# microsoft/DirectXTex

Hardware: AMD Instinct MI355X
Metric: Mtexels/s BC7 encode (4096^2 RGBA8, TEX_COMPRESS_DEFAULT) (higher is better)
Workload: dtype fp32 seed fit + i32 exact error sums (u8 texels in, 128-bit blocks out); 1 GPU; cfg2: 4096x4096 RGBA8 -> BC7_UNORM, TEX_COMPRESS_DEFAULT, one image per GPU, source and payload resident in HBM (dxtex_compress_device)

## Files before the change

### directxtex_amd/csrc/bc6h_encode.hip

```cpp
#include "dxtex_kernels.h"
#include "bc67_tables.h"
#include "bc7_core.h"
#include "bc6h_core.h"
#include "search_common.h"
#include <algorithm>
#include <cstdlib>
#include <cstdio>
#include <vector>

namespace dxtex
{
namespace
{
using namespace bc6h;

struct Ep16 { uint32_t a01, a2b0, b12; };
__device__ __forceinline__ Ep16 pack_ep16(const int (&A)[3], const int (&B)[3])
{
    Ep16 e;
    e.a01 = (uint32_t(A[0]) & 0xFFFFu) | (uint32_t(A[1]) << 16);
    e.a2b0 = (uint32_t(A[2]) & 0xFFFFu) | (uint32_t(B[0]) << 16);
    e.b12 = (uint32_t(B[1]) & 0xFFFFu) | (uint32_t(B[2]) << 16);
    return e;
}
// ... 976 lines not shown
        const uint32_t myTask = a.order[idx].x;
        const Rec6 rec = a.recs[myTask];
        const uint32_t nb = myTask % a.nblocks;
        const int prec = a.prec1[myTask / a.nblocks];
        const float* gp = a.fpix + uint64_t(nb) * 48 + (lane & 15);
        const float tr = gp[0], tg = gp[16], tb = gp[32];
        EndPts e;
        unpack_ep16(rec.ep, sg, e.A, e.B);
        Perturb6 st = perturb6_begin(e, rec.err);
        while (st.ch < 3)
        {
            float err; int v;
            perturb6_wave_macro(tr, tg, tb, lane, st, prec, sg, err, v);
            st = perturb6_transition(st, err, v);
        }
        if (lane == 0)
        {
            a.recs[myTask].ep = pack_ep16(st.ep.A, st.ep.B);
            { const float mk = ep16_mark(sg, st.ep.A, st.ep.B); if (mk < 0.0f) a.recs[myTask].err = mk; }
        }
    }
}

__global__ void __launch_bounds__(256) bc6h_store_kernel(Bc6hArgs a)
{
    const uint32_t nb = blockIdx.x * 256u + threadIdx.x;
    if (nb >= a.nblocks) return;
    const Best6 b = a.best[nb];
    const BcSeg& im = seg_of(a.seg, nb);
    const uint32_t gb = im.nb0 + (nb - im.l0);
    const uint32_t by = gb / im.nbw, bx = gb - by * im.nbw;
    uint64_t* out = reinterpret_cast<uint64_t*>(im.dst + uint64_t(by) * im.dstRowPitch) + 2 * uint64_t(bx);
    out[0] = b.lo; out[1] = b.hi;
}

const uint64_t kMaxBlocksPerPass6 = dev_env("DXTEX_MAX_BLOCKS_PER_PASS") ? std::max<uint64_t>(1, strtoull(dev_env("DXTEX_MAX_BLOCKS_PER_PASS"), nullptr, 10)) : (1u << 22);
struct Scratch6
{
    size_t fpix, lists, seeds, recs, orgs, order, tinfo, counters, best, bounds, recs1, orgs1, order1, tinfo1, counters1, opts, total;
    explicit Scratch6(uint64_t nb)
    {
        auto up = [](size_t v) { return (v + 255) & ~size_t(255); };
        size_t o = 0;
        fpix = o; o = up(o + nb * 48 * sizeof(float));
        lists = o; o = up(o + nb * 8);
        seeds = o; o = up(o + nb * SEED_INTS * sizeof(int));
        recs = o; o = up(o + nb * 16 * sizeof(Rec6));
        orgs = o; o = up(o + nb * 16 * sizeof(OrgSave));
        order = o; o = up(o + nb * 16 * sizeof(uint2));
        tinfo = o; o = up(o + nb * 16 * sizeof(uint32_t));
        counters = o; o = up(o + 128 * sizeof(uint32_t));
        best = o; o = up(o + nb * sizeof(Best6));
        bounds = o; o = up(o + nb * 17 * sizeof(float));
        recs1 = o; o = up(o + nb * 4 * sizeof(Rec6));
        orgs1 = o; o = up(o + nb * 4 * sizeof(OrgSave));
        order1 = o; o = up(o + nb * 4 * sizeof(uint2));
        tinfo1 = o; o = up(o + nb * 4 * sizeof(uint32_t));
        counters1 = o; o = up(o + 128 * sizeof(uint32_t));
        opts = o; o = up(o + nb * 16 * sizeof(OptSave));
        total = o;
    }
};
}

size_t bc6h_scratch_bytes(uint64_t nblocks, size_t nimages)
{
    return Scratch6(nblocks < kMaxBlocksPerPass6 ? nblocks : kMaxBlocksPerPass6).total + seg_table_bytes(nblocks, kMaxBlocksPerPass6, nimages);
}

hipError_t launch_bc6h_encode(const SrcView& src, uint8_t* dst, uint64_t dstRowPitch, bool isSigned, void* scratch,
                              hipStream_t stream, KernelMarks* marks, const SideStreams* side)
{
    BcImage one; one.src = src; one.dst = dst; one.dstRowPitch = dstRowPitch;
    return launch_bc6h_encode_many(&one, 1, isSigned, scratch, stream, marks, side);
}

hipError_t launch_bc6h_encode_many(const BcImage* images, size_t count, bool isSigned, void* scratch, hipStream_t stream, KernelMarks* marks,
                                   const SideStreams* side)
{
#define DXTEX_MARK(NAME) do { if (marks) marks->mark(NAME); } while (0)
    std::vector<BcSeg> segs;
    std::vector<BcPass> passes;
    uint64_t perPass = 0;
    if (!build_passes(images, count, kMaxBlocksPerPass6, segs, passes, &perPass)) return hipSuccess;
    const Scratch6 L(perPass);
    uint8_t* base = static_cast<uint8_t*>(scratch);
    BcSeg* dSegs = reinterpret_cast<BcSeg*>(base + L.total);
    const hipError_t ce = upload_segments(dSegs, segs, passes, stream);
    if (ce != hipSuccess) return ce;
    for (const BcPass& pass : passes)
    {
        Bc6hArgs a;
        set_pass(a.seg, dSegs, segs, pass);
        a.nblocks = pass.nblocks;
        a.isSigned = isSigned ? 1 : 0;
        static const bool noPrune = dev_env("DXTEX_BC6H_NO_PRUNE") != nullptr;
        a.prune = noPrune ? 0 : 1;
        a.fpix = reinterpret_cast<float*>(base + L.fpix);
        a.lists = base + L.lists;
        a.seeds = reinterpret_cast<int*>(base + L.seeds);
        a.recs = reinterpret_cast<Rec6*>(base + L.recs);
        a.orgs = reinterpret_cast<OrgSave*>(base + L.orgs);
        a.order = reinterpret_cast<uint2*>(base + L.order);
        a.tinfo = reinterpret_cast<uint32_t*>(base + L.tinfo);
        a.counters = reinterpret_cast<uint32_t*>(base + L.counters);
        a.best = reinterpret_cast<Best6*>(base + L.best);
        a.bounds = reinterpret_cast<float*>(base + L.bounds);
        a.opts = reinterpret_cast<OptSave*>(base + L.opts);
        a.saveOpt = 0;
        a.boundsReady = 0;
        a.filterStats = 0;
        a.mode = ModeRt();

        DXTEX_MARK("bc6h_rough");
        hipLaunchKernelGGL(bc6h_rough_kernel, dim3((a.nblocks + 3) / 4), dim3(256), 0, stream, a);
        DXTEX_MARK("bc6h_block_seed");
        hipLaunchKernelGGL(bc6h_block_seed_kernel, dim3((a.nblocks + 255) / 256), dim3(256), 0, stream, a);
        if (dev_env("DXTEX_BC6H_DUMP"))
        {
            (void)hipStreamSynchronize(stream);
            const uint32_t n = std::min<uint32_t>(a.nblocks, 4);
            std::vector<uint8_t> l(n * 8); std::vector<int> sd(n * SEED_INTS);
            (void)hipMemcpy(l.data(), a.lists, l.size(), hipMemcpyDeviceToHost);
            (void)hipMemcpy(sd.data(), a.seeds, sd.size() * 4, hipMemcpyDeviceToHost);
            for (uint32_t b = 0; b < n; ++b)
            {
                fprintf(stderr, "block %u shapes:", b);
                for (int i = 0; i < 8; ++i) fprintf(stderr, " %d", l[b * 8 + i]);
                fprintf(stderr, "\n  seeds rank0:");
                for (int i = 0; i < 12; ++i) fprintf(stderr, " %d", sd[b * SEED_INTS + i]);
                fprintf(stderr, "\n");
            }
        }
        static const int onlyMode = dev_env("DXTEX_BC6H_ONLY_MODE") ? atoi(dev_env("DXTEX_BC6H_ONLY_MODE")) : -1;
        static const bool noSearch = dev_env("DXTEX_BC6H_NO_SEARCH") != nullptr;
        static const Bc6hMode kModes[14] = {
            { 0x00, 1, 1, 3, { 10, 10, 10 }, { 5, 5, 5 } }, { 0x01, 1, 1, 3, { 7, 7, 7 }, { 6, 6, 6 } }, { 0x02, 1, 1, 3, { 11, 11, 11 }, { 5, 4, 4 } },
            { 0x06, 1, 1, 3, { 11, 11, 11 }, { 4, 5, 4 } }, { 0x0a, 1, 1, 3, { 11, 11, 11 }, { 4, 4, 5 } }, { 0x0e, 1, 1, 3, { 9, 9, 9 }, { 5, 5, 5 } },
            { 0x12, 1, 1, 3, { 8, 8, 8 }, { 6, 5, 5 } }, { 0x16, 1, 1, 3, { 8, 8, 8 }, { 5, 6, 5 } }, { 0x1a, 1, 1, 3, { 8, 8, 8 }, { 5, 5, 6 } },
            { 0x1e, 1, 0, 3, { 6, 6, 6 }, { 6, 6, 6 } }, { 0x03, 0, 0, 4, { 10, 10, 10 }, { 10, 10, 10 } }, { 0x07, 0, 1, 4, { 11, 11, 11 }, { 9, 9, 9 } },
            { 0x0b, 0, 1, 4, { 12, 12, 12 }, { 8, 8, 8 } }, { 0x0f, 0, 1, 4, { 16, 16, 16 }, { 4, 4, 4 } } };
        auto set_mode_on = [&](Bc6hArgs& a, int mi)
        {
            const Bc6hMode& k = kModes[mi];
            a.mode.index = mi; a.mode.code = k.code; a.mode.regions2 = k.regions2; a.mode.transformed = k.transformed; a.mode.prec = k.prec[0];
            for (int c = 0; c < 3; ++c) a.mode.delta[c] = k.delta[c];
        };
        auto set_mode = [&](int mi) { set_mode_on(a, mi); };
        auto sort_tasks = [&](const Bc6hArgs& a, uint32_t ntasks, hipStream_t stream)
        {
            const uint32_t binGroups = std::min<uint32_t>(kBinGroups, (ntasks + 255) / 256);
            (void)hipMemsetAsync(a.counters, 0, 128 * sizeof(uint32_t), stream);
            hipLaunchKernelGGL(bc7_bin_count_kernel, dim3(binGroups), dim3(256), 0, stream, a.tinfo, ntasks, a.counters);
            hipLaunchKernelGGL(bc7_bin_scan_kernel, dim3(1), dim3(1), 0, stream, a.counters);
            hipLaunchKernelGGL(bc7_bin_scatter_kernel, dim3(binGroups), dim3(256), 0, stream, a.tinfo, ntasks, a.counters, a.order);
        };
        a.taskBase = 0;
        for (int m = 0; m < 4; ++m) a.prec1[m] = kModes[10 + m].prec[0];
        static const std::vector<int> order6 = []
        {
            std::vector<int> o;
            const char* e = dev_env("DXTEX_BC6H_ORDER");
            const char* p = e ? e : DXTEX_BC6H_DEFAULT_ORDER;
            while (*p) { if (*p >= '0' && *p <= '9') o.push_back(int(strtol(p, const_cast<char**>(&p), 10))); else ++p; }
            return o;
        }();
        int prevPrec = -1;
        a.samePrec = 0;
        std::vector<int> run2;
        for (int mi : order6) if (mi >= 0 && mi <= 9 && (onlyMode < 0 || mi == onlyMode)) run2.push_back(mi);
        static const int forkBack = dev_env("DXTEX_BC6H_FORK_BACK") ? atoi(dev_env("DXTEX_BC6H_FORK_BACK")) : 2;
        const SideStreams* fork = (marks || forkBack <= 0 || run2.size() < size_t(forkBack) + 1 || onlyMode >= 0) ? nullptr : side;
        Bc6hArgs a1 = a;
        a1.recs = reinterpret_cast<Rec6*>(base + L.recs1);
        a1.orgs = reinterpret_cast<OrgSave*>(base + L.orgs1);
        a1.order = reinterpret_cast<uint2*>(base + L.order1);
        a1.tinfo = reinterpret_cast<uint32_t*>(base + L.tinfo1);
        a1.counters = reinterpret_cast<uint32_t*>(base + L.counters1);
        a1.samePrec = 0;
        auto one_region_search = [&](hipStream_t stream, KernelMarks* marks)
        {
            const uint32_t gridPP = (a1.nblocks + 255) / 256;
            DXTEX_MARK("bc6h_pre_1region");
            a1.boundsReady = 0;
            for (int m = 0; m < 4; ++m)
            {
                if (onlyMode >= 0 && 10 + m != onlyMode) continue;
                set_mode_on(a1, 10 + m); a1.taskBase = uint32_t(m) * a1.nblocks;
                hipLaunchKernelGGL(bc6h_pre_kernel<0>, dim3(gridPP), dim3(256), 0, stream, a1);
                a1.boundsReady = 1;
            }
            const uint32_t ntasks = a1.nblocks * 4u;
            if (onlyMode >= 0)
                for (int m = 0; m < 4; ++m) if (10 + m != onlyMode) (void)hipMemsetAsync(a1.tinfo + uint64_t(m) * a1.nblocks, 0, uint64_t(a1.nblocks) * 4, stream);
            DXTEX_MARK("bc6h_bin_1region");
            sort_tasks(a1, ntasks, stream);
            DXTEX_MARK("bc6h_perturb_1region");
            static const uint32_t waveMax = dev_env("DXTEX_BC6H_WAVE_MAX") ? uint32_t(strtoul(dev_env("DXTEX_BC6H_WAVE_MAX"), nullptr, 0)) : kWaveTaskMax6;
            if (!noSearch)
            {
                hipLaunchKernelGGL(bc6h_perturb_kernel<16>, dim3(std::min<uint32_t>(kSearchWaves, (ntasks + 63) / 64)), dim3(64), 0, stream, a1, waveMax);
                hipLaunchKernelGGL(bc6h_perturb_wave_kernel, dim3(std::min<uint32_t>(kSearchWaves, ntasks)), dim3(64), 0, stream, a1, waveMax);
            }
        };
        bool forked = false;
        for (size_t at = 0; at < run2.size(); ++at)
        {
            const int mi = run2[at];
            if (fork && at + size_t(forkBack) == run2.size())
            {
                (void)hipEventRecord(fork->forked, stream);
                (void)hipStreamWaitEvent(fork->side[0], fork->forked, 0);
                one_region_search(fork->side[0], nullptr);
                (void)hipEventRecord(fork->joined[0], fork->side[0]);
                forked = true;
            }
            set_mode(mi);
            static const bool noReuse = dev_env("DXTEX_BC6H_NO_REUSE") != nullptr;
            a.samePrec = (!noReuse && prevPrec == kModes[mi].prec[0]) ? 1 : 0;
            prevPrec = kModes[mi].prec[0];
            a.saveOpt = (!noReuse && at + 1 < run2.size() && kModes[run2[at + 1]].prec[0] == kModes[mi].prec[0]) ? 1 : 0;
            const uint32_t ntasks = a.nblocks * 16u;
            const uint32_t gridPP = (a.nblocks + 15) / 16;
            static const char* const kPre[10] = { "bc6h_pre_m0", "bc6h_pre_m1", "bc6h_pre_m2", "bc6h_pre_m3", "bc6h_pre_m4", "bc6h_pre_m5", "bc6h_pre_m6", "bc6h_pre_m7", "bc6h_pre_m8", "bc6h_pre_m9" };
            static const char* const kPerturb[10] = { "bc6h_perturb_m0", "bc6h_perturb_m1", "bc6h_perturb_m2", "bc6h_perturb_m3", "bc6h_perturb_m4", "bc6h_perturb_m5", "bc6h_perturb_m6", "bc6h_perturb_m7", "bc6h_perturb_m8", "bc6h_perturb_m9" };
            static const char* const kPost[10] = { "bc6h_post_m0", "bc6h_post_m1", "bc6h_post_m2", "bc6h_post_m3", "bc6h_post_m4", "bc6h_post_m5", "bc6h_post_m6", "bc6h_post_m7", "bc6h_post_m8", "bc6h_post_m9" };
            DXTEX_MARK(kPre[mi]);
            hipLaunchKernelGGL(bc6h_pre_kernel<1>, dim3(gridPP), dim3(256), 0, stream, a);
            a.boundsReady = 1;
            DXTEX_MARK("bc6h_bin_2region");
            sort_tasks(a, ntasks, stream);
#if defined(DXTEX_DEV)
            static const bool stats6 = dev_env("DXTEX_BC6H_STATS") != nullptr;
            a.filterStats = stats6 ? 1 : 0;
            if (stats6)
            {
                uint32_t c[40] = {};
                (void)hipStreamSynchronize(stream);
                (void)hipMemcpy(c, a.counters, sizeof(c), hipMemcpyDeviceToHost);
                std::fprintf(stderr, "bc6h stats mode %d (prec %d): %u task slots, %u live (16-texel: %u)\n", mi, a.mode.prec, ntasks, c[34], c[16]);
            }
#endif
            DXTEX_MARK(kPerturb[mi]);
            static const bool plainPerturb = dev_env("DXTEX_BC6H_PERTURB_PLAIN") != nullptr;
            if (!noSearch)
            {
                const dim3 grid(std::min<uint32_t>(kSearchWaves, (ntasks + 63) / 64));
                if (plainPerturb) hipLaunchKernelGGL(bc6h_perturb_kernel<8>, grid, dim3(64), 0, stream, a, 0u);
                else if (isSigned) hipLaunchKernelGGL(bc6h_perturb_filter_kernel<true>, grid, dim3(64), 0, stream, a);
                else hipLaunchKernelGGL(bc6h_perturb_filter_kernel<false>, grid, dim3(64), 0, stream, a);
            }
#if defined(DXTEX_DEV)
            if (stats6 && !plainPerturb)
            {
                uint32_t c[24] = {};
                (void)hipStreamSynchronize(stream);
                (void)hipMemcpy(c, a.counters + 64, sizeof(c), hipMemcpyDeviceToHost);
                auto u64 = [&](int i) { unsigned long long v = 0; memcpy(&v, c + i, 8); return double(v); };
                const double tk = u64(10), tx = u64(8), tb = u64(12), tl = u64(14), tr = u64(16), tp = u64(18), tm = u64(20);
                const double lanesMacro = c[4] ? double(c[5]) / c[4] : 0.0, lanesBound = c[0] ? double(c[7]) / c[0] : 0.0, lanesRounds = c[3] ? double(c[6]) / c[3] : 0.0,
                             lanesList = c[1] ? double(c[2]) / c[1] : 0.0;
                std::fprintf(stderr, "bc6h filter mode %d: %u macros (%.1f lanes active), %u pair steps, %u with passing candidates (%.2f per such step), %u list rounds; "
                             "exact evaluation %.1f %% of the waves' time\n", mi, c[4], lanesMacro, c[0], c[1], lanesList, c[3], tk ? 100.0 * tx / tk : 0.0);
                const double tOtherMacro = tm - tb - tx, tRest = tk - tm - tp, tBack = tx - tl - tr;
                const double weighted = (tb * lanesBound + tl * lanesList + tr * lanesRounds + tBack * lanesList + tOtherMacro * lanesMacro + tp * 32.0 + tRest * lanesMacro) / (tk ? tk : 1.0);
                std::fprintf(stderr, "bc6h filter sections mode %d | share of wave time, lanes busy: bound loops %.1f %% at %.1f | list write %.1f %% at %.1f | exact rounds %.1f %% at %.1f | "
                             "read-back + syncs %.1f %% at %.1f | rest of PerturbOne (fixed palettes, bound setup, transitions) %.1f %% at %.1f | task pickup %.1f %% | outside %.1f %% | "
                             "time-weighted lanes %.1f of 64\n", mi, 100 * tb / tk, lanesBound, 100 * tl / tk, lanesList, 100 * tr / tk, lanesRounds, 100 * tBack / tk, lanesList,
                             100 * tOtherMacro / tk, lanesMacro, 100 * tp / tk, 100 * tRest / tk, weighted);
            }
#endif
            DXTEX_MARK(kPost[mi]);
            hipLaunchKernelGGL(bc6h_post_kernel<1>, dim3(gridPP), dim3(256), 0, stream, a);
        }
        if (forked) (void)hipStreamWaitEvent(stream, fork->joined[0], 0);
        else one_region_search(stream, marks);
        {
            const uint32_t gridPP = (a1.nblocks + 255) / 256;
            DXTEX_MARK("bc6h_post_1region");
            for (int m = 0; m < 4; ++m)
            {
                if (onlyMode >= 0 && 10 + m != onlyMode) continue;
                set_mode_on(a1, 10 + m); a1.taskBase = uint32_t(m) * a1.nblocks;
                hipLaunchKernelGGL(bc6h_post_kernel<0>, dim3(gridPP), dim3(256), 0, stream, a1);
            }
        }
        DXTEX_MARK("bc6h_store");
        hipLaunchKernelGGL(bc6h_store_kernel, dim3((a.nblocks + 255) / 256), dim3(256), 0, stream, a);
    }
    DXTEX_MARK(nullptr);
#undef DXTEX_MARK
    return hipGetLastError();
}
}
```

### directxtex_amd/csrc/bc7_encode.hip

```cpp
#include "dxtex_kernels.h"
#include "bc67_tables.h"
#include "bc7_core.h"
#include "search_common.h"
#include <algorithm>
#include <cstdio>
#include <cstdlib>
#include <vector>

namespace dxtex
{
namespace
{
using namespace bc7;

struct Cand { uint32_t err; uint32_t ord; uint64_t lo, hi; };

enum : int { SLOT_M0 = 0, SLOT_M1, SLOT_M2, SLOT_M3, SLOT_M4A, SLOT_M4B, SLOT_M5, SLOT_M6, SLOT_M7, NUM_SLOTS };
enum : int { LIST_BYTES = 64 };

enum : int { PHASE_ALL = 0, PHASE_EARLY = 1, PHASE_LATE = 2 };

struct Bc7Args
{
    SegTable seg;
// ... 1189 lines not shown
            atomicMin(&a.bestErr[nb], err);
        }
        else if (!active && rank == 0 && mine)
        {
            Cand c; c.err = 0xFFFFFFFFu; c.ord = 0xFFFFFFFFu; c.lo = 0; c.hi = 0;
            a.cands[uint64_t(nb) * NUM_SLOTS + TM::SLOT] = c;
        }
    }
}

template<bool RGBA>
__global__ void __launch_bounds__(256) bc7_block_seeds_kernel(Bc7Args a)
{
    const uint32_t nb = blockIdx.x * 256u + threadIdx.x;
    if (nb >= a.nblocks) return;
    const BcSeg& sg = seg_of(a.seg, nb);
    float f[64];
#pragma unroll
    for (int t = 0; t < 16; ++t) { uint32_t ldr; load_block_texel(sg.src, sg.nbw, sg.nb0 + (nb - sg.l0), uint32_t(t), &f[t * 4], ldr); }
    uint32_t A, B;
    seed_endpoints<RGBA, true>(f, 0xFFFFu, A, B);
    a.seeds1[uint64_t(nb) * 2 + (RGBA ? 1 : 0)] = make_uint2(A, B);
}

__global__ void __launch_bounds__(256) bc7_flag_count_kernel(Bc7Args a, uint32_t* out)
{
    uint32_t n = 0, m = 0;
    for (uint32_t nb = blockIdx.x * 256u + threadIdx.x; nb < a.nblocks; nb += gridDim.x * 256u)
    {
        uint8_t* lst = a.lists + uint64_t(nb) * LIST_BYTES;
        const bool hasAlpha = lst[32] != 0;
        bool first = hasAlpha;
        if (!first)
        {
            const uint4* px4 = reinterpret_cast<const uint4*>(a.px + uint64_t(nb) * 16);
            const uint4 q0 = px4[0], q1 = px4[1], q2 = px4[2], q3 = px4[3];
            const uint32_t px[16] = { q0.x, q0.y, q0.z, q0.w, q1.x, q1.y, q1.z, q1.w, q2.x, q2.y, q2.z, q2.w, q3.x, q3.y, q3.z, q3.w };
            const int ea = *reinterpret_cast<const int*>(lst + 56);
            first = int64_t(subset_lower_bound(px, 0xFFFFu, 0u, 4)) * 100 <= int64_t(ea) * a.early6Pct;
        }
        lst[37] = first ? 1 : 0;
        n += first ? 1u : 0u;
        m += hasAlpha ? 1u : 0u;
    }
#pragma unroll
    for (int o = 32; o > 0; o >>= 1) { n += __shfl_xor(n, o); m += __shfl_xor(m, o); }
    if ((threadIdx.x & 63u) == 0 && n) atomicAdd(out, n);
    if ((threadIdx.x & 63u) == 0 && m) atomicAdd(out + 1, m);
}

__global__ void __launch_bounds__(256) bc7_texels_kernel(Bc7Args a)
{
    const uint32_t i = blockIdx.x * 256u + threadIdx.x;
    if (i >= a.nblocks * 16u) return;
    float f4[4]; uint32_t ldr;
    const BcSeg& sg = seg_of(a.seg, i >> 4);
    load_block_texel(sg.src, sg.nbw, sg.nb0 + ((i >> 4) - sg.l0), i & 15u, f4, ldr);
    a.px[i] = ldr;
    if ((i & 15u) == 0) { a.zeroOrd[i >> 4] = 0xFFFFFFFFu; a.bestErr[i >> 4] = 0x7FFFFFFF; }
}

__global__ void __launch_bounds__(256) bc7_pick_kernel(Bc7Args a, uint32_t slotMask)
{
    const uint32_t nb = blockIdx.x * 256u + threadIdx.x;
    if (nb >= a.nblocks) return;
    const Cand* c = a.cands + uint64_t(nb) * NUM_SLOTS;
    uint64_t bestKey = ~0ull;
    uint64_t lo = 0, hi = 0;
#pragma unroll
    for (int s = 0; s < NUM_SLOTS; ++s)
    {
        if (!((slotMask >> s) & 1u)) continue;
        if (s == SLOT_M7 && a.flagged[1] == 0) continue;
        const Cand v = c[s];
        if (v.err == 0xFFFFFFFFu) continue;
        const uint64_t key = (uint64_t(v.err) << 32) | v.ord;
        if (key < bestKey) { bestKey = key; lo = v.lo; hi = v.hi; }
    }
    const BcSeg& sg = seg_of(a.seg, nb);
    const uint32_t gb = sg.nb0 + (nb - sg.l0);
    const uint32_t by = gb / sg.nbw, bx = gb - by * sg.nbw;
    uint64_t* out = reinterpret_cast<uint64_t*>(sg.dst + uint64_t(by) * sg.dstRowPitch) + 2 * uint64_t(bx);
    out[0] = lo; out[1] = hi;
}
}

namespace
{
const uint64_t kMaxBlocksPerPass = dev_env("DXTEX_MAX_BLOCKS_PER_PASS") ? std::max<uint64_t>(1, strtoull(dev_env("DXTEX_MAX_BLOCKS_PER_PASS"), nullptr, 10)) : (1u << 22);
constexpr int kMaxTasksPerBlock = 64;
const uint64_t kSmallPassBlocks = dev_env("DXTEX_BC7_SMALL_BLOCKS") ? strtoull(dev_env("DXTEX_BC7_SMALL_BLOCKS"), nullptr, 10) : 262144;
struct ScratchLayout
{
    size_t lists, cands, px, recs, order, tinfo, counters, zeroOrd, bestErr, seeds, seeds1, seeds3, flagcnt, auxRecs, auxOrder, auxTinfo, auxCounters, total;
    size_t auxTpb, auxSlices;
    explicit ScratchLayout(uint64_t nb, bool threeSubsets)
    {
        auto up = [](size_t v) { return (v + 255) & ~size_t(255); };
        const size_t tpb = threeSubsets ? kMaxTasksPerBlock : 32;
        const bool small = nb <= kSmallPassBlocks;
        auxTpb = small ? tpb : 4; auxSlices = small ? size_t(kSideStreams) : 2;
        size_t o = 0;
        lists = o; o = up(o + nb * LIST_BYTES);
        cands = o; o = up(o + nb * NUM_SLOTS * sizeof(Cand));
        px = o; o = up(o + nb * 64);
        recs = o; o = up(o + nb * tpb * sizeof(TaskRec));
        order = o; o = up(o + nb * tpb * sizeof(uint2));
        tinfo = o; o = up(o + nb * tpb * sizeof(uint32_t));
        counters = o; o = up(o + 64 * sizeof(uint32_t));
        zeroOrd = o; o = up(o + nb * sizeof(uint32_t));
        bestErr = o; o = up(o + nb * sizeof(int));
        seeds = o; o = up(o + nb * 64 * sizeof(uint2));
        seeds1 = o; o = up(o + nb * 2 * sizeof(uint2));
        seeds3 = o; o = up(o + (threeSubsets ? nb * 192 * sizeof(uint2) : 0));
        flagcnt = o; o = up(o + 256);
        auxRecs = o; o = up(o + auxSlices * nb * auxTpb * sizeof(TaskRec));
        auxOrder = o; o = up(o + auxSlices * nb * auxTpb * sizeof(uint2));
        auxTinfo = o; o = up(o + auxSlices * nb * auxTpb * sizeof(uint32_t));
        auxCounters = o; o = up(o + size_t(kSideStreams) * 64 * sizeof(uint32_t));
        total = o;
    }
};

template<int MODE, int IM>
void launch_mode(const Bc7Args& a0, hipStream_t stream, KernelMarks* marks, const char* const (&names)[7])
{
    typedef TaskMap<MODE, IM> TM;
    constexpr int BPW = (TM::TPB >= 64) ? 1 : 64 / TM::TPB;
    const uint32_t nb = a0.nblocks;
    const uint32_t ntasks = nb * uint32_t(TM::TPB);
    const uint32_t gridPP = (nb + 4 * BPW - 1) / (4 * BPW);
    constexpr bool kWhole = TM::NS == 1;
    constexpr uint32_t kExhMax = (MODE == 6) ? kWaveTaskMax : kWaveTaskMax45;
    static const bool noGroup = dev_env("DXTEX_BC7_NO_GROUP") != nullptr;
    const bool maybeShortP = kWhole && !noGroup && (MODE == 6 || ntasks <= 4u * kPerturbWaveMax);
    const bool maybeShortE = kWhole && !noGroup && (MODE == 6 || ntasks <= 4u * kExhMax);
    const uint32_t wavesP = std::min<uint32_t>(kSearchWaves, (ntasks + 1) / 2), wavesE = std::min<uint32_t>(kSearchWaves, ntasks);
    Bc7Args a = a0;
    a.gate = nullptr; a.gateMin = 0;
    if (a0.flagged && !(a0.flags & BCF_BC7_QUICK))
    {
        if (MODE == 7) { a.gate = a0.flagged + 1; a.gateMin = 1; }
        else if (a0.phase == PHASE_EARLY && (MODE == 4 || MODE == 5)) { a.gate = a0.flagged + 1; a.gateMin = std::max<uint32_t>(1u, a0.earlyAlphaMin); }
        else if (a0.phase == PHASE_EARLY && MODE == 6) { a.gate = a0.flagged; a.gateMin = std::max<uint32_t>(1u, a0.early6Min); }
    }
    a.perturbWaveMax = maybeShortP ? kPerturbWaveMax : 0u;
    a.exhWaveMax = maybeShortE ? kExhMax : 0u;
    if (marks) marks->mark(names[0]);
    hipLaunchKernelGGL((bc7_pre_kernel<MODE, IM>), dim3(gridPP), dim3(256), 0, stream, a);
    if (marks) marks->mark(names[1]);
    (void)hipMemsetAsync(a.counters, 0, 64 * sizeof(uint32_t), stream);
    const uint32_t binGroups = std::min<uint32_t>(kBinGroups, (ntasks + 255) / 256);
    hipLaunchKernelGGL(bc7_bin_count_kernel, dim3(binGroups), dim3(256), 0, stream, a.tinfo, ntasks, a.counters, a.gate, a.gateMin);
    hipLaunchKernelGGL(bc7_bin_scan_kernel, dim3(1), dim3(1), 0, stream, a.counters);
    hipLaunchKernelGGL(bc7_bin_scatter_kernel, dim3(binGroups), dim3(256), 0, stream, a.tinfo, ntasks, a.counters, a.order, a.gate, a.gateMin);
    if (marks) marks->mark(names[2]);
    const uint32_t waves = std::min<uint32_t>(kSearchWaves, (ntasks + 63) / 64);
    static const int tailBelow = dev_env("DXTEX_BC7_TAIL_BELOW") ? atoi(dev_env("DXTEX_BC7_TAIL_BELOW")) : 48;
    static const bool perturbPlain = dev_env("DXTEX_BC7_PERTURB_PLAIN") != nullptr;
    static const int rangeTests = dev_env("DXTEX_BC7_NO_PEEL") ? 3 : ((dev_env("DXTEX_BC7_RANGE_TESTS") ? atoi(dev_env("DXTEX_BC7_RANGE_TESTS")) & 0xFF : DXTEX_RANGE_TESTS) |
                                                                       ((dev_env("DXTEX_BC7_PEEL_LAYERS") ? atoi(dev_env("DXTEX_BC7_PEEL_LAYERS")) : 1) << 8));
    if constexpr (PaletteBits<MODE, IM>::AB == 0)
    {
        if constexpr (MODE == 1 || MODE == 6)
        {
            if (perturbPlain) hipLaunchKernelGGL((bc7_perturb_kernel<MODE, IM, CH_ALL>), dim3(waves), dim3(64), 0, stream, a, 0);
            else hipLaunchKernelGGL((bc7_perturb_filter_kernel<MODE, IM, CH_ALL>), dim3(waves), dim3(64), 0, stream, a, 0);
        }
        else
            hipLaunchKernelGGL((bc7_perturb_kernel<MODE, IM, CH_ALL>), dim3(waves), dim3(64), 0, stream, a, 0);
        if constexpr (kWhole) { if (maybeShortP) hipLaunchKernelGGL((bc7_perturb_wave_kernel<MODE, IM, CH_ALL>), dim3(wavesP), dim3(64), 0, stream, a); }
        if (marks) marks->mark(names[4]);
        if constexpr (kWhole) { if (maybeShortE) hipLaunchKernelGGL((bc7_exhaustive_wave_kernel<MODE, IM, CH_ALL>), dim3(wavesE), dim3(64), 0, stream, a); }
        hipLaunchKernelGGL((bc7_exhaustive_kernel<MODE, IM, CH_ALL>), dim3(waves), dim3(64), 0, stream, a, 1, tailBelow, rangeTests);
    }
    else
    {
        if constexpr (MODE == 4 && IM == 1 && DXTEX_PF_M4 != 0)
        {
            if (perturbPlain) hipLaunchKernelGGL((bc7_perturb_kernel<MODE, IM, CH_COLOR>), dim3(waves), dim3(64), 0, stream, a, 0);
            else hipLaunchKernelGGL((bc7_perturb_filter_kernel<MODE, IM, CH_COLOR>), dim3(waves), dim3(64), 0, stream, a, 0);
        }
        else
            hipLaunchKernelGGL((bc7_perturb_kernel<MODE, IM, CH_COLOR>), dim3(waves), dim3(64), 0, stream, a, 0);
        if (maybeShortP) hipLaunchKernelGGL((bc7_perturb_wave_kernel<MODE, IM, CH_COLOR>), dim3(wavesP), dim3(64), 0, stream, a);
        if (marks) marks->mark(names[3]);
        hipLaunchKernelGGL((bc7_perturb_kernel<MODE, IM, CH_ALPHA>), dim3(waves), dim3(64), 0, stream, a, 1);
        if (maybeShortP) hipLaunchKernelGGL((bc7_perturb_wave_kernel<MODE, IM, CH_ALPHA>), dim3(wavesP), dim3(64), 0, stream, a);
        if (marks) marks->mark(names[4]);
        if (maybeShortE) hipLaunchKernelGGL((bc7_exhaustive_wave_kernel<MODE, IM, CH_COLOR>), dim3(wavesE), dim3(64), 0, stream, a);
        hipLaunchKernelGGL((bc7_exhaustive_kernel<MODE, IM, CH_COLOR>), dim3(waves), dim3(64), 0, stream, a, 2, tailBelow, rangeTests);
        if (marks) marks->mark(names[5]);
        if (maybeShortE) hipLaunchKernelGGL((bc7_exhaustive_wave_kernel<MODE, IM, CH_ALPHA>), dim3(wavesE), dim3(64), 0, stream, a);
        hipLaunchKernelGGL((bc7_exhaustive_kernel<MODE, IM, CH_ALPHA>), dim3(waves), dim3(64), 0, stream, a, 3, tailBelow, rangeTests);
    }
    if (marks) marks->mark(names[6]);
    hipLaunchKernelGGL((bc7_post_kernel<MODE, IM>), dim3(gridPP), dim3(256), 0, stream, a);
#if defined(DXTEX_DEV)
    static const bool stats = dev_env("DXTEX_BC7_STATS") != nullptr;
    if (stats)
    {
        uint32_t c[40] = {};
        (void)hipStreamSynchronize(stream);
        (void)hipMemcpy(c, a.counters, sizeof(c), hipMemcpyDeviceToHost);
        std::fprintf(stderr, "bc7 stats %-22s phase %d: %9u task slots, %9u live; by size 16..1:", names[0], a.phase, ntasks, c[34]);
        for (int b = 16; b >= 1; --b) std::fprintf(stderr, " %u", c[b]);
        std::fprintf(stderr, "\n");
    }
#endif
}
}

#if defined(DXTEX_BC7_WAVETIMES)
namespace
{
void bc7_wavetimes_report()
{
    (void)hipDeviceSynchronize();
    static int call = 0;
    static const int wanted = dev_env("DXTEX_BC7_WT_CALL") ? atoi(dev_env("DXTEX_BC7_WT_CALL")) : 2;
    const bool print = call++ == wanted;
    static std::vector<unsigned long long> h(size_t(WT_KEYS) * 8192 * WT_FIELDS);
    static std::vector<unsigned int> hist(size_t(WT_KEYS) * 256);
    (void)hipMemcpyFromSymbol(h.data(), HIP_SYMBOL(g_wt), h.size() * 8);
    (void)hipMemcpyFromSymbol(hist.data(), HIP_SYMBOL(g_wtHist), hist.size() * 4);
    unsigned long long tAll = ~0ull;
    for (size_t i = 0; i < size_t(WT_KEYS) * 8192; ++i) if (h[i * WT_FIELDS + 2]) tAll = std::min(tAll, h[i * WT_FIELDS]);
    static const char* const kinds[3] = { "perturb", "perturb_filter", "exhaustive" };
    for (int key = 0; key < WT_KEYS; ++key)
    {
        const unsigned long long* w = h.data() + size_t(key) * 8192 * WT_FIELDS;
        std::vector<unsigned long long> st, dr, en; unsigned long long rounds = 0, lanes = 0, life = 0, maxR = 0, tasks = 0, maxT = 0;
        for (int i = 0; i < 8192; ++i)
            if (w[i * WT_FIELDS + 2])
            {
                st.push_back(w[i * WT_FIELDS]); dr.push_back(w[i * WT_FIELDS + 1]); en.push_back(w[i * WT_FIELDS + 2]);
                rounds += w[i * WT_FIELDS + 3]; lanes += w[i * WT_FIELDS + 4]; tasks += w[i * WT_FIELDS + 5];
                life += w[i * WT_FIELDS + 2] - w[i * WT_FIELDS]; maxR = std::max(maxR, w[i * WT_FIELDS + 3]); maxT = std::max(maxT, w[i * WT_FIELDS + 5]);
            }
        if (st.empty() || !print) continue;
        const unsigned long long t0 = *std::min_element(st.begin(), st.end()), t1 = *std::max_element(en.begin(), en.end());
        std::sort(st.begin(), st.end()); std::sort(dr.begin(), dr.end()); std::sort(en.begin(), en.end());
        const double dur = double(t1 - t0); const size_t n = st.size();
        auto pct = [&](const std::vector<unsigned long long>& v, double p) { return 100.0 * double(v[std::min(n - 1, size_t(p * n))] - t0) / dur; };
        const unsigned int* hh = hist.data() + size_t(key) * 256;
        unsigned long long nt = 0, rt = 0; for (int r = 0; r < 256; ++r) { nt += hh[r]; rt += (unsigned long long)hh[r] * r; }
        auto hp = [&](double p) { unsigned long long c = 0; for (int r = 0; r < 256; ++r) { c += hh[r]; if (double(c) >= p * double(nt)) return r; } return 255; };
        unsigned long long rLong = 0; for (int r = 2 * hp(0.9) + 1; r < 256; ++r) if (r >= 0) rLong += (unsigned long long)hh[r] * r;
        const int chset = key % 3, im = (key / 3) % 2, mode = (key / 6) % 8, kind = key / 48;
        std::fprintf(stderr, "wt %s<%d,%d,%d>: at %.2f ms, span %.3f ms, %zu wavefronts worked; starts p50 %.0f p90 %.0f; saw the queue drained p10 %.0f p50 %.0f p90 %.0f; ends p10 %.0f p50 %.0f p90 %.0f p99 %.0f (%% of span); "
                     "mean lifetime %.0f %%; rounds / wavefront mean %.1f max %llu, busy lanes / round %.1f; tasks / wavefront mean %.0f max %llu; "
                     "finished tasks %llu, rounds / task mean %.2f p50 %d p90 %d p99 %d p99.9 %d, share of task-rounds in tasks above 2 x p90: %.1f %%\n",
                     kinds[kind], mode, im, chset, double(t0 - tAll) / 1e5, dur / 1e5, n, pct(st, 0.5), pct(st, 0.9), pct(dr, 0.1), pct(dr, 0.5), pct(dr, 0.9),
                     pct(en, 0.1), pct(en, 0.5), pct(en, 0.9), pct(en, 0.99), 100.0 * double(life) / (dur * n), double(rounds) / n, maxR, rounds ? double(lanes) / rounds : 0.0,
                     double(tasks) / n, maxT, nt, nt ? double(rt) / nt : 0.0, hp(0.5), hp(0.9), hp(0.99), hp(0.999), rt ? 100.0 * double(rLong) / rt : 0.0);
        std::vector<int> idx; for (int i = 0; i < 8192; ++i) if (w[i * WT_FIELDS + 2]) idx.push_back(i);
        std::sort(idx.begin(), idx.end(), [&](int x, int y) { return w[x * WT_FIELDS + 2] > w[y * WT_FIELDS + 2]; });
        for (size_t k = 0; k < std::min<size_t>(4, idx.size()); ++k)
        {
            const unsigned long long* e = w + idx[k] * WT_FIELDS;
            std::fprintf(stderr, "    late wavefront %d: start %.0f drained %.0f end %.0f %% of span, rounds %llu, busy lanes / round %.1f, tasks %llu\n", idx[k],
                         100.0 * double(e[0] - t0) / dur, 100.0 * double(e[1] - t0) / dur, 100.0 * double(e[2] - t0) / dur, e[3], e[3] ? double(e[4]) / e[3] : 0.0, e[5]);
        }
        {
            const unsigned long long* e = w + idx[idx.size() / 2] * WT_FIELDS;
            std::fprintf(stderr, "    median wavefront %d: start %.0f drained %.0f end %.0f %% of span, rounds %llu, busy lanes / round %.1f, tasks %llu\n", idx[idx.size() / 2],
                         100.0 * double(e[0] - t0) / dur, 100.0 * double(e[1] - t0) / dur, 100.0 * double(e[2] - t0) / dur, e[3], e[3] ? double(e[4]) / e[3] : 0.0, e[5]);
        }
    }
    std::fill(h.begin(), h.end(), 0ull); std::fill(hist.begin(), hist.end(), 0u);
    (void)hipMemcpyToSymbol(HIP_SYMBOL(g_wt), h.data(), h.size() * 8);
    (void)hipMemcpyToSymbol(HIP_SYMBOL(g_wtHist), hist.data(), hist.size() * 4);
}
}
#endif

size_t bc7_scratch_bytes(uint64_t nblocks, uint32_t flags, size_t nimages)
{
    const bool three = (flags & BCF_USE_3SUBSETS) != 0;
    size_t need = ScratchLayout(nblocks < kMaxBlocksPerPass ? nblocks : kMaxBlocksPerPass, three).total;
    if (nblocks > kSmallPassBlocks) need = std::max(need, ScratchLayout(kSmallPassBlocks, three).total);
    return need + seg_table_bytes(nblocks, kMaxBlocksPerPass, nimages);
}

hipError_t launch_bc7_encode(const SrcView& src, uint8_t* dst, uint64_t dstRowPitch, uint32_t flags,
                             void* scratch, hipStream_t stream, KernelMarks* marks, const SideStreams* side)
{
    BcImage one; one.src = src; one.dst = dst; one.dstRowPitch = dstRowPitch;
    return launch_bc7_encode_many(&one, 1, flags, scratch, stream, marks, side);
}

hipError_t launch_bc7_encode_many(const BcImage* images, size_t count, uint32_t flags, void* scratch, hipStream_t stream, KernelMarks* marks,
                                  const SideStreams* side)
{
#define DXTEX_MARK(NAME) do { if (marks) marks->mark(NAME); } while (0)
#define DXTEX_MODE(MODE, IM, TAG) do { static const char* const n_[7] = { "bc7_pre_" TAG, "bc7_bin_" TAG, "bc7_perturb_" TAG, "bc7_perturb_alpha_" TAG, \
                                           "bc7_exhaustive_" TAG, "bc7_exhaustive_alpha_" TAG, "bc7_post_" TAG }; \
                                       launch_mode<MODE, IM>(a, stream, marks, n_); } while (0)
    std::vector<BcSeg> segs;
    std::vector<BcPass> passes;
    uint64_t perPass = 0;
    if (!build_passes(images, count, kMaxBlocksPerPass, segs, passes, &perPass)) return hipSuccess;
    const bool three = (flags & BCF_USE_3SUBSETS) != 0;
    const ScratchLayout L(perPass, three);
    uint8_t* base = static_cast<uint8_t*>(scratch);
    BcSeg* dSegs = reinterpret_cast<BcSeg*>(base + L.total);
    const hipError_t ce = upload_segments(dSegs, segs, passes, stream);
// ... 177 lines not shown
```

### directxtex_amd/csrc/search_common.h

```cpp
#pragma once
#include <hip/hip_runtime.h>
#include <stdint.h>
#include <algorithm>
#include <cstring>
#include <vector>
#include "dxtex_kernels.h"

namespace dxtex
{
namespace
{
struct BcSeg
{
    SrcView src;
    uint8_t* dst;
    uint64_t dstRowPitch;
    uint32_t nbw;
    uint32_t nb0;
    uint32_t l0;
    uint32_t pad;
};

struct SegTable
{
    BcSeg inl[2];
    const BcSeg* segs;
    uint32_t nseg;
};

__device__ __forceinline__ const BcSeg& seg_of(const SegTable& t, uint32_t local)
{
    if (t.nseg <= 2) return (t.nseg == 2 && t.inl[1].l0 <= local) ? t.inl[1] : t.inl[0];
    uint32_t lo = 0, hi = t.nseg;
    while (hi - lo > 1) { const uint32_t mid = (lo + hi) >> 1; if (t.segs[mid].l0 <= local) lo = mid; else hi = mid; }
    return t.segs[lo];
}

struct BcPass { uint32_t seg0, nseg, nblocks; };

inline uint64_t build_passes(const BcImage* images, size_t count, uint64_t maxPerPass, std::vector<BcSeg>& segs, std::vector<BcPass>& passes, uint64_t* perPassOut)
{
    uint64_t total = 0;
    for (size_t i = 0; i < count; ++i) total += uint64_t((images[i].src.width + 3) / 4) * ((images[i].src.height + 3) / 4);
    const uint64_t perPass = total < maxPerPass ? total : maxPerPass;
    *perPassOut = perPass;
    if (!total) return 0;
    BcPass cur = { 0, 0, 0 };
    for (size_t i = 0; i < count; ++i)
    {
        const uint32_t nbw = (images[i].src.width + 3) / 4, nbh = (images[i].src.height + 3) / 4;
        uint64_t left = uint64_t(nbw) * nbh, at = 0;
        while (left)
        {
            const uint64_t take = std::min<uint64_t>(left, perPass - cur.nblocks);
            BcSeg sg; sg.src = images[i].src; sg.dst = images[i].dst; sg.dstRowPitch = images[i].dstRowPitch;
            sg.nbw = nbw; sg.nb0 = uint32_t(at); sg.l0 = cur.nblocks; sg.pad = 0;
            segs.push_back(sg);
            ++cur.nseg; cur.nblocks += uint32_t(take); at += take; left -= take;
            if (cur.nblocks == perPass) { passes.push_back(cur); cur = { uint32_t(segs.size()), 0, 0 }; }
        }
    }
    if (cur.nblocks) passes.push_back(cur);
    return total;
}

inline hipError_t upload_segments(BcSeg* dSegs, std::vector<BcSeg>& segs, const std::vector<BcPass>& passes, hipStream_t stream)
{
    bool needTable = false;
    for (const BcPass& pass : passes) needTable |= pass.nseg > 2;
    if (!needTable) return hipSuccess;
    struct Staging { void* host = nullptr; size_t capacity = 0; hipEvent_t consumed = nullptr; bool pending = false; int device = -1; };
    static thread_local Staging st;
    int device = 0;
    hipError_t e = hipGetDevice(&device);
    if (e != hipSuccess) return e;
    if (st.pending) { e = hipEventSynchronize(st.consumed); if (e != hipSuccess) return e; st.pending = false; }
    const size_t bytes = segs.size() * sizeof(BcSeg);
    if (st.device != device || st.capacity < bytes)
    {
        if (st.host) (void)hipHostFree(st.host);
        if (st.consumed) (void)hipEventDestroy(st.consumed);
        st = Staging();
        e = hipHostMalloc(&st.host, std::max<size_t>(bytes, 4096), hipHostMallocDefault);
        if (e != hipSuccess) return e;
        e = hipEventCreateWithFlags(&st.consumed, hipEventDisableTiming);
        if (e != hipSuccess) return e;
        st.capacity = std::max<size_t>(bytes, 4096); st.device = device;
    }
    std::memcpy(st.host, segs.data(), bytes);
    e = hipMemcpyAsync(dSegs, st.host, bytes, hipMemcpyHostToDevice, stream);
    if (e != hipSuccess) return e;
    e = hipEventRecord(st.consumed, stream);
    st.pending = (e == hipSuccess);
    return e;
}

inline void set_pass(SegTable& t, const BcSeg* dSegs, const std::vector<BcSeg>& segs, const BcPass& pass)
{
    t.segs = dSegs + pass.seg0; t.nseg = pass.nseg;
    t.inl[0] = segs[pass.seg0]; t.inl[1] = segs[pass.seg0 + (pass.nseg > 1 ? 1 : 0)];
}

inline size_t seg_table_bytes(uint64_t nblocks, uint64_t maxPerPass, size_t nimages)
{
    const uint64_t perPass = nblocks < maxPerPass ? nblocks : maxPerPass;
    const uint64_t passes = perPass ? (nblocks + perPass - 1) / perPass : 1;
    return ((nimages + passes + 1) * sizeof(BcSeg) + 255) & ~size_t(255);
}

__device__ __forceinline__ void wave_lds_sync()
{
    __builtin_amdgcn_fence(__ATOMIC_RELEASE, "wavefront");
    __builtin_amdgcn_wave_barrier();
    __builtin_amdgcn_fence(__ATOMIC_ACQUIRE, "wavefront");
}

__device__ __forceinline__ int wave_prefix_min(int v)
{
    v = min(v, __builtin_amdgcn_update_dpp(v, v, 0x111, 0xF, 0xF, false));
    v = min(v, __builtin_amdgcn_update_dpp(v, v, 0x112, 0xF, 0xF, false));
    v = min(v, __builtin_amdgcn_update_dpp(v, v, 0x114, 0xF, 0xF, false));
    v = min(v, __builtin_amdgcn_update_dpp(v, v, 0x118, 0xF, 0xF, false));
    v = min(v, __builtin_amdgcn_update_dpp(v, v, 0x142, 0xA, 0xF, false));
    v = min(v, __builtin_amdgcn_update_dpp(v, v, 0x143, 0xC, 0xF, false));
    return v;
}

__device__ __forceinline__ void selection_pass(int& e, uint32_t& s, int lane, int i)
{
    const int v = (lane >= i) ? e : 0x7FFFFFFF;
    const int incl = wave_prefix_min(v);
    int excl = __builtin_amdgcn_update_dpp(0x7FFFFFFF, incl, 0x138, 0xF, 0xF, false);
    if (lane <= i) excl = 0x7FFFFFFF;
    const bool isrec = (lane > i) && (e < excl);
    const unsigned long long mask = __ballot(isrec);
    int srcLane = lane;
    if (isrec)
    {
        const unsigned long long below = mask & ((1ull << lane) - 1ull);
        srcLane = below ? (63 - __clzll(below)) : i;
    }
    else if (lane == i && mask)
        srcLane = 63 - __clzll(mask);
    e = __shfl(e, srcLane);
    s = uint32_t(__shfl(int(s), srcLane));
}

constexpr int kBinGroups = 2048;

__global__ void __launch_bounds__(256) bc7_bin_count_kernel(const uint32_t* tinfo, uint32_t ntasks, uint32_t* counters, const uint32_t* gate = nullptr, uint32_t gateMin = 0)
{
    if (gate && *gate < gateMin) return;
    __shared__ uint32_t hist[17];
    if (threadIdx.x < 17) hist[threadIdx.x] = 0;
    __syncthreads();
    const uint32_t per = (ntasks + gridDim.x - 1) / gridDim.x;
    const uint32_t t0 = blockIdx.x * per, t1 = min(ntasks, t0 + per);
    for (uint32_t t = t0 + threadIdx.x; t < t1; t += 256)
    {
        const uint32_t np = tinfo[t] >> 24;
        if (np) atomicAdd(&hist[np], 1u);
    }
    __syncthreads();
    if (threadIdx.x >= 1 && threadIdx.x <= 16 && hist[threadIdx.x]) atomicAdd(&counters[threadIdx.x], hist[threadIdx.x]);
}

__global__ void bc7_bin_scan_kernel(uint32_t* counters)
{
    if (threadIdx.x != 0 || blockIdx.x != 0) return;
    uint32_t run = 0;
    for (int b = 16; b >= 1; --b) { counters[17 + b] = run; run += counters[b]; }
    counters[34] = run;
}

__global__ void __launch_bounds__(256) bc7_bin_scatter_kernel(const uint32_t* tinfo, uint32_t ntasks, uint32_t* counters, uint2* order, const uint32_t* gate = nullptr, uint32_t gateMin = 0)
{
    if (gate && *gate < gateMin) return;
    __shared__ uint32_t hist[17], cursor[17];
    if (threadIdx.x < 17) hist[threadIdx.x] = 0;
    __syncthreads();
    const uint32_t per = (ntasks + gridDim.x - 1) / gridDim.x;
    const uint32_t t0 = blockIdx.x * per, t1 = min(ntasks, t0 + per);
    for (uint32_t t = t0 + threadIdx.x; t < t1; t += 256)
    {
        const uint32_t np = tinfo[t] >> 24;
        if (np) atomicAdd(&hist[np], 1u);
    }
    __syncthreads();
    if (threadIdx.x >= 1 && threadIdx.x <= 16)
        cursor[threadIdx.x] = hist[threadIdx.x] ? atomicAdd(&counters[17 + threadIdx.x], hist[threadIdx.x]) : 0u;
    __syncthreads();
    for (uint32_t t = t0 + threadIdx.x; t < t1; t += 256)
    {
        const uint32_t ti = tinfo[t], np = ti >> 24;
        if (np) order[atomicAdd(&cursor[np], 1u)] = make_uint2(t, ti);
    }
}

constexpr int kQueueBase = 36;
constexpr int kSearchWaves = 8192;

constexpr uint32_t kQueueBatch = 128;

struct WaveQueue
{
    uint32_t lo, hi;
    bool drained;
};

__device__ __forceinline__ uint32_t queue_take(WaveQueue& q, uint32_t* head, uint32_t live, unsigned long long idle, int lane)
{
    if (q.lo >= q.hi && !q.drained)
    {
        const uint32_t batch = (live > uint32_t(kSearchWaves) * 64u) ? kQueueBatch : 64u;
        uint32_t base = 0;
        if (lane == 0) base = atomicAdd(head, batch);
        base = uint32_t(__builtin_amdgcn_readfirstlane(int(base)));
        q.lo = base;
        q.hi = min(base + batch, live);
        if (base >= live) { q.drained = true; q.hi = q.lo; }
    }
    const uint32_t k = uint32_t(__popcll(idle & ((1ull << lane) - 1ull)));
    const uint32_t avail = q.hi - q.lo;
    const uint32_t mine = (((idle >> lane) & 1ull) && k < avail) ? (q.lo + k) : 0xFFFFFFFFu;
    q.lo += min(uint32_t(__popcll(idle)), avail);
    return mine;
}

}
}
```

Measured before the change: 136.5 Mtexels/s.

## Fold bin prefix scan into scatter and use wave-ballot histograms

```diff
diff --git a/directxtex_amd/csrc/bc6h_encode.hip b/directxtex_amd/csrc/bc6h_encode.hip
--- a/directxtex_amd/csrc/bc6h_encode.hip
+++ b/directxtex_amd/csrc/bc6h_encode.hip
@@ -1152,7 +1152,6 @@
             const uint32_t binGroups = std::min<uint32_t>(kBinGroups, (ntasks + 255) / 256);
             (void)hipMemsetAsync(a.counters, 0, 128 * sizeof(uint32_t), stream);
             hipLaunchKernelGGL(bc7_bin_count_kernel, dim3(binGroups), dim3(256), 0, stream, a.tinfo, ntasks, a.counters);
-            hipLaunchKernelGGL(bc7_bin_scan_kernel, dim3(1), dim3(1), 0, stream, a.counters);
             hipLaunchKernelGGL(bc7_bin_scatter_kernel, dim3(binGroups), dim3(256), 0, stream, a.tinfo, ntasks, a.counters, a.order);
         };
         a.taskBase = 0;
diff --git a/directxtex_amd/csrc/bc7_encode.hip b/directxtex_amd/csrc/bc7_encode.hip
--- a/directxtex_amd/csrc/bc7_encode.hip
+++ b/directxtex_amd/csrc/bc7_encode.hip
@@ -1365,7 +1365,6 @@
     (void)hipMemsetAsync(a.counters, 0, 64 * sizeof(uint32_t), stream);
     const uint32_t binGroups = std::min<uint32_t>(kBinGroups, (ntasks + 255) / 256);
     hipLaunchKernelGGL(bc7_bin_count_kernel, dim3(binGroups), dim3(256), 0, stream, a.tinfo, ntasks, a.counters, a.gate, a.gateMin);
-    hipLaunchKernelGGL(bc7_bin_scan_kernel, dim3(1), dim3(1), 0, stream, a.counters);
     hipLaunchKernelGGL(bc7_bin_scatter_kernel, dim3(binGroups), dim3(256), 0, stream, a.tinfo, ntasks, a.counters, a.order, a.gate, a.gateMin);
     if (marks) marks->mark(names[2]);
     const uint32_t waves = std::min<uint32_t>(kSearchWaves, (ntasks + 63) / 64);
diff --git a/directxtex_amd/csrc/search_common.h b/directxtex_amd/csrc/search_common.h
--- a/directxtex_amd/csrc/search_common.h
+++ b/directxtex_amd/csrc/search_common.h
@@ -148,52 +148,125 @@
 
 constexpr int kBinGroups = 2048;
 
+struct BinSlice { uint32_t s0, s1, steps; };
+
+__device__ __forceinline__ BinSlice bin_slice(uint32_t ntasks)
+{
+    const uint32_t per = (ntasks + gridDim.x - 1) / gridDim.x, perWave = (per + 3) / 4;
+    const uint32_t t0 = min(ntasks, blockIdx.x * per), t1 = min(ntasks, t0 + per);
+    BinSlice s;
+    s.s0 = min(t1, t0 + (threadIdx.x >> 6) * perWave);
+    s.s1 = min(t1, s.s0 + perWave);
+    s.steps = (perWave + 63) / 64;
+    return s;
+}
+
+constexpr uint32_t kBinBatch = 4;
+
+__device__ __forceinline__ void load_batch(const uint32_t* tinfo, uint32_t t, uint32_t s1, uint32_t (&ti)[kBinBatch])
+{
+#pragma unroll
+    for (uint32_t j = 0; j < kBinBatch; ++j) ti[j] = (t + 64 * j < s1) ? tinfo[t + 64 * j] : 0u;
+}
+
+__device__ __forceinline__ void wave_histogram(const uint32_t* tinfo, const BinSlice& s, uint32_t (&cnt)[17])
+{
+#pragma unroll
+    for (int b = 1; b <= 16; ++b) cnt[b] = 0;
+    uint32_t t = s.s0 + (threadIdx.x & 63);
+    for (uint32_t k = 0; k < s.steps; k += kBinBatch, t += 64 * kBinBatch)
+    {
+        uint32_t ti[kBinBatch];
+        load_batch(tinfo, t, s.s1, ti);
+#pragma unroll
+        for (uint32_t j = 0; j < kBinBatch; ++j)
+        {
+            const uint32_t np = ti[j] >> 24;
+            if (__ballot(np != 0) == 0) continue;
+#pragma unroll
+            for (int b = 1; b <= 16; ++b) cnt[b] += uint32_t(__popcll(__ballot(np == uint32_t(b))));
+        }
+    }
+}
+
+__device__ __forceinline__ void share_histogram(const uint32_t (&cnt)[17], uint32_t (&wcnt)[4][17])
+{
+    const uint32_t lane = threadIdx.x & 63;
+    uint32_t mine = 0;
+#pragma unroll
+    for (int b = 1; b <= 16; ++b) if (lane == uint32_t(b)) mine = cnt[b];
+    if (lane >= 1 && lane <= 16) wcnt[threadIdx.x >> 6][lane] = mine;
+    __syncthreads();
+}
+
 __global__ void __launch_bounds__(256) bc7_bin_count_kernel(const uint32_t* tinfo, uint32_t ntasks, uint32_t* counters, const uint32_t* gate = nullptr, uint32_t gateMin = 0)
 {
     if (gate && *gate < gateMin) return;
-    __shared__ uint32_t hist[17];
-    if (threadIdx.x < 17) hist[threadIdx.x] = 0;
+    __shared__ uint32_t wcnt[4][17];
+    uint32_t cnt[17];
+    wave_histogram(tinfo, bin_slice(ntasks), cnt);
+    share_histogram(cnt, wcnt);
+    if (threadIdx.x >= 1 && threadIdx.x <= 16)
+    {
+        const uint32_t n = wcnt[0][threadIdx.x] + wcnt[1][threadIdx.x] + wcnt[2][threadIdx.x] + wcnt[3][threadIdx.x];
+        if (n) atomicAdd(&counters[threadIdx.x], n);
+    }
+}
+
+__global__ void __launch_bounds__(256) bc7_bin_scatter_kernel(const uint32_t* tinfo, uint32_t ntasks, uint32_t* counters, uint2* order, const uint32_t* gate = nullptr, uint32_t gateMin = 0)
+{
+    if (gate && *gate < gateMin) return;
+    __shared__ uint32_t wcnt[4][17], first[17];
+    const uint32_t lane = threadIdx.x & 63, wave = threadIdx.x >> 6;
+    const bool binLane = lane >= 1 && lane <= 16;
+    const uint32_t total = binLane ? counters[lane] : 0u;
+    const BinSlice s = bin_slice(ntasks);
+    uint32_t cnt[17];
+    wave_histogram(tinfo, s, cnt);
+    share_histogram(cnt, wcnt);
+    uint32_t start = 0, live = 0;
+#pragma unroll
+    for (int b = 1; b <= 16; ++b)
+    {
+        const uint32_t n = uint32_t(__builtin_amdgcn_readlane(int(total), b));
+        live += n;
+        if (lane < uint32_t(b)) start += n;
+    }
+    if (blockIdx.x == 0 && threadIdx.x == 0) counters[34] = live;
+    if (threadIdx.x >= 1 && threadIdx.x <= 16)
+    {
+        const uint32_t n = wcnt[0][lane] + wcnt[1][lane] + wcnt[2][lane] + wcnt[3][lane];
+        first[lane] = start + (n ? atomicAdd(&counters[17 + lane], n) : 0u);
+    }
     __syncthreads();
-    const uint32_t per = (ntasks + gridDim.x - 1) / gridDim.x;
-    const uint32_t t0 = blockIdx.x * per, t1 = min(ntasks, t0 + per);
-    for (uint32_t t = t0 + threadIdx.x; t < t1; t += 256)
-    {
-        const uint32_t np = tinfo[t] >> 24;
-        if (np) atomicAdd(&hist[np], 1u);
-    }
-    __syncthreads();
-    if (threadIdx.x >= 1 && threadIdx.x <= 16 && hist[threadIdx.x]) atomicAdd(&counters[threadIdx.x], hist[threadIdx.x]);
-}
-
-__global__ void bc7_bin_scan_kernel(uint32_t* counters)
-{
-    if (threadIdx.x != 0 || blockIdx.x != 0) return;
-    uint32_t run = 0;
-    for (int b = 16; b >= 1; --b) { counters[17 + b] = run; run += counters[b]; }
-    counters[34] = run;
-}
-
-__global__ void __launch_bounds__(256) bc7_bin_scatter_kernel(const uint32_t* tinfo, uint32_t ntasks, uint32_t* counters, uint2* order, const uint32_t* gate = nullptr, uint32_t gateMin = 0)
-{
-    if (gate && *gate < gateMin) return;
-    __shared__ uint32_t hist[17], cursor[17];
-    if (threadIdx.x < 17) hist[threadIdx.x] = 0;
-    __syncthreads();
-    const uint32_t per = (ntasks + gridDim.x - 1) / gridDim.x;
-    const uint32_t t0 = blockIdx.x * per, t1 = min(ntasks, t0 + per);
-    for (uint32_t t = t0 + threadIdx.x; t < t1; t += 256)
-    {
-        const uint32_t np = tinfo[t] >> 24;
-        if (np) atomicAdd(&hist[np], 1u);
-    }
-    __syncthreads();
-    if (threadIdx.x >= 1 && threadIdx.x <= 16)
-        cursor[threadIdx.x] = hist[threadIdx.x] ? atomicAdd(&counters[17 + threadIdx.x], hist[threadIdx.x]) : 0u;
-    __syncthreads();
-    for (uint32_t t = t0 + threadIdx.x; t < t1; t += 256)
-    {
-        const uint32_t ti = tinfo[t], np = ti >> 24;
-        if (np) order[atomicAdd(&cursor[np], 1u)] = make_uint2(t, ti);
+    uint32_t next = 0;
+    if (binLane)
+    {
+        next = first[lane];
+        for (uint32_t w = 0; w < wave; ++w) next += wcnt[w][lane];
+    }
+    uint32_t t = s.s0 + lane;
+    for (uint32_t k = 0; k < s.steps; k += kBinBatch, t += 64 * kBinBatch)
+    {
+        uint32_t ti[kBinBatch];
+        load_batch(tinfo, t, s.s1, ti);
+#pragma unroll
+        for (uint32_t j = 0; j < kBinBatch; ++j)
+        {
+            const uint32_t np = ti[j] >> 24;
+            if (__ballot(np != 0) == 0) continue;
+            unsigned long long same = ~0ull;
+#pragma unroll
+            for (int bit = 0; bit < 5; ++bit)
+            {
+                const int mine = (int(np) << (31 - bit)) >> 31;
+                same &= ~(__ballot(mine != 0) ^ (unsigned long long)(long long)mine);
+            }
+            const uint32_t rank = __builtin_amdgcn_mbcnt_hi(uint32_t(same >> 32), __builtin_amdgcn_mbcnt_lo(uint32_t(same), 0u));
+            const uint32_t at = uint32_t(__builtin_amdgcn_ds_bpermute(int(np << 2), int(next)));
+            next += uint32_t(__builtin_amdgcn_ds_permute(int(np << 2), __popcll(same)));
+            if (np) order[at + rank] = make_uint2(t + 64 * j, ti[j]);
+        }
     }
 }
 
```

New measurement: 136.8 Mtexels/s (median of 6 runs). Within noise of the previous version (+0.2%).
